# acados/acados

Measured on AMD Instinct MI355X. Metric: OCP-QP solves/sec (batch) at N=50 nx=8 nu=3, higher is better.
Workload: dtype f64; 1 GPU; random LQR OCP-QP (BASELINE configs[1]): N=50 nx=8 nu=3, u-box + x0 equality, full-space Riccati IPM, cold start, tol 1e-8, iter_max 50; batch_per_gpu=65536, global_batch=65536, parallelism=instance-sharded x1, kernel=1tpi-box<NX=8,NU=3,XBOX=0>

## Files before the change

acados_amd/csrc/gpu_batch.hip:

```cpp
#include <hip/hip_runtime.h>

#include <stdio.h>
#include <stdlib.h>
#include <string.h>

#include <algorithm>
#include <functional>
#include <string>
#include <climits>
#include <vector>

#include "acados_amd/ocp_qp_gpu_batch.h"
#include "gpu_ipm_internal.h"
#include "ipm_kernels.hpp"
#include "ipm_kernels_box.hpp"
#include "ipm_kernels_box_small.hpp"
#include "ipm_kernels_wpi.hpp"
#include "ipm_kernels_w16.hpp"
#include "ipm_kernels_w16r.hpp"
#include "ipm_kernels_w16t.hpp"
#include "ipm_kernels_wpi_mfma.hpp"
#include "res_kernels.hpp"
#include "pcond_kernels_w16.hpp"
#include "pcond_kernels_mfma.hpp"
// ... 77 lines not shown
{
    ocp_qp_gpu_batch *c = nullptr;
    int *d_list = nullptr;
    int list_cap = 0;
    int cap = 0;
};

enum BlobKind { BLOB_IN, BLOB_OUT, BLOB_VEC, BLOB_SEED, BLOB_KINDS };
struct BulkMap
{
    bool built = false;
    int len = 0, nm = 0;
    std::vector<std::string> fields;
    std::vector<int> seg_stage, seg_off, seg_len;
    std::vector<int> arr, elem;
    int *d_arr = nullptr, *d_elem = nullptr, *d_moff = nullptr, *d_mstage = nullptr, *d_mbit = nullptr;
    int *d_sgn = nullptr, *d_elem2 = nullptr;
    int *d_arr_g = nullptr, *d_elem_g = nullptr;
    gqp::GArrTable T;
};

struct HeldDynamics
{
    int tiles_invariant = 0, fact_launches = 0, rhs_launches = 0;
    hipEvent_t ev = nullptr;
    ocp_qp_gpu_batch *b = nullptr;
    bool enabled = false;
    bool polish = false;
    enum { DETECTING, AWAITING, COUNTED } state = COUNTED;
    int tiles = 0;

    void begin(ocp_qp_gpu_batch *root, hipStream_t s, bool polish_loop);
    int bits(bool affine_sweep = false) const { return !enabled ? 0 : (affine_sweep && state == DETECTING) ? 3 : 1; }
    void after_detect(hipStream_t s);
    void before_factor();
    void count();
    bool all_held() const;
    void end(hipStream_t s);
};

struct ocp_qp_gpu_batch
{
    int B = 0, Bp = 0, N = 0, device = 0;
    std::vector<int> nx, nu, nbx, nbu, nb, ng, ns, nbxe;
    std::vector<std::vector<int>> idxb, idxs_rev, idxe;
    std::vector<std::vector<int>> perm;
    bool finalized = false;
    bool use_box = false;
    int aos = 0;
    int AW = 1;
    int wpi = 0;
    bool wpi_mfma = false;
    int w16 = 0;
    size_t shmem = 0;
    size_t shmem_fwd = 0;
    size_t shmem_fact = 0;
    bool w16_soft = false;
    int w16_ng = 0;
    KernelSet wpi_ks;
    int w16_slots = 0;
    size_t w16_shmem = 0;
// ... 60 lines not shown
    int cond_N = 0;
    int cond_keep_iterate = 0;
    int force_NX = 0, force_NU = 0;
    std::vector<int> user_blocks;
    int pcond_state = 0;
    ocp_qp_gpu_batch *child = nullptr;
    const PcondSet *pc = nullptr;
    int pc_rt = 0;
    int pc_lane_expand = 0;
    const PcondzSet *pcz = nullptr;
    int pcz_mfma = 1;
    size_t pc_shmem = 0;
    std::vector<int> blk_start;
    gqp::PcondMap pmap;
    double time_xcond = 0.0;
    bool lhs_ready = false;
    SubBatch sub[SUB_ROLES];
    const KernelSet *force_ks = nullptr;
    int compact_min = 1 << 30;
    int tail_max = 12288;
    int tail_div = 4;
    int n_tail_switches = 0;
    int hold_dynamics = 1;
    HeldDynamics held;
    bool factor_stale = false;
    bool sens_open = false;
    GArr sfix = {nullptr, 0, 0};
    int *d_saved_status = nullptr;
    int ric_alg = 1;
    struct Ric1
    {
        bool saved = false;
        KernelSet own_ks;
        int w16 = 0;
        kern_redo_t w16_solve = nullptr;
        bool wpi_mfma = false;
        size_t shmem = 0, shmem_fwd = 0, shmem_fact = 0;
        std::string kname;
    } ric1;
    int n_compactions = 0;
    gqp::ResOut R = {{nullptr, 0, 0}, {nullptr, 0, 0}, {nullptr, 0, 0}, {nullptr, 0, 0}, {nullptr, 0, 0}, nullptr, 0};
    BulkMap blob[BLOB_KINDS];
    struct GradMap
    {
        bool built = false;
        int len = 0, olen = 0;
// ... 246 lines not shown
    D.t = garr<double>(b, (size_t) ((o_ct + RP)));
    D.rg = garr<double>(b, (size_t) ((N + 1) * n));
    D.rgs = garr<double>(b, (size_t) (o_s));
    D.rb = garr<double>(b, (size_t) ((N + 1) * NX));
    D.rd = garr<double>(b, (size_t) ((o_ct + RP)));
    D.rm = garr<double>(b, (size_t) ((o_ct + RP)));
    D.dux = garr<double>(b, (size_t) ((N + 2) * n));
    D.dsv = garr<double>(b, (size_t) (o_s));
    D.dpi = garr<double>(b, (size_t) ((N + 2) * NX));
    D.dlam = garr<double>(b, (size_t) ((o_ct + RP)));
    D.dt = garr<double>(b, (size_t) ((o_ct + RP)));
    D.pcorr = garr<double>(b, (size_t) ((o_ct + RP)));
    D.sD = garr<double>(b, (size_t) (o_s));
    D.sR = garr<double>(b, (size_t) (o_s));
    D.Lf = garr<double>(b, (size_t) ((N + 1) * NP));
    D.lf = garr<double>(b, (size_t) ((N + 1) * n));
    D.res = dalloc<double>(b, 4 * Bp);
    D.mu = dalloc<double>(b, Bp); D.smu = dalloc<double>(b, Bp);
    D.alpha = dalloc<double>(b, Bp); D.obj = dalloc<double>(b, Bp);
    D.apend = dalloc<double>(b, Bp);
    D.iter = dalloc<int>(b, Bp); D.status = dalloc<int>(b, Bp);
    D.n_active = dalloc<int>(b, 1);
    D.tile_inv = dalloc<int>(b, (size_t) Bp / 64);
    b->stat_inst = b->B < 64 ? b->B : 64;
    b->stat_rows = 0;
    D.stat = nullptr; D.stat_inst = 0; D.stat_rows = 0;
    D.perm = nullptr; D.n_perm = 0;

    const int grid = (b->B + 63) / 64;
    for (int k = 0; k <= N; k++)
    {
        for (int j = 0; j < n; j++)
        {
            const bool real = j < NU ? j < b->nu[k] : (j - NU) < b->nx[k];
            if (!real)
                hipLaunchKernelGGL(gqp::k_fill_strided, dim3(grid), dim3(64), 0, b->stream, D.RSQ, 1.0, b->B,
                                   k * NP + PK(j, j));
        }
        const GqpStage &S = b->st[k];
        const int nbg = S.nb + S.ng, nct = 2 * nbg + 2 * S.ns;
        uint64_t m[2] = {0, 0};
        for (int e = 0; e < nct; e++) m[e >> 6] |= (uint64_t) 1 << (e & 63);
        for (size_t e = 0; e < b->idxe[k].size(); e++)
        {
            const int sp = b->perm[k][b->idxe[k][e]];
            m[sp >> 6] &= ~((uint64_t) 1 << (sp & 63));
// ... 507 lines not shown
        std::vector<int> map, map2;
        GArr arr = {nullptr, 0, 0}, arr2 = {nullptr, 0, 0};
        const size_t flen = strlen(f);
        if (flen > 5 && !strcmp(f + flen - 5, "_mask"))
        {
            const int len = mask_bits(b, f, k, map);
            if (len < 0) { rc = -1; break; }
            if (len == 0) continue;
            if (src_len != len) { src = stage_in(b, data, (size_t) b->B * len, is_device); src_len = len; }
            int *dm = upload_map(b, map);
            hipLaunchKernelGGL(gqp::k_setmask, dim3(grid), dim3(64), 0, b->stream, src, b->B, len, dm, b->D.amask, k, b->AW);
            continue;
        }
        const int len = field_map(b, f, k, map, &arr, &map2, &arr2);
        if (len < 0)
        {
            if (stage < 0) continue;
            rc = -1;
            break;
        }
        if (len == 0) continue;
        if (src_len != len) { src = stage_in(b, data, (size_t) b->B * len, is_device); src_len = len; }
        int *dm = upload_map(b, map);
        hipLaunchKernelGGL(gqp::k_scatter, dim3(grid), dim3(64), 0, b->stream, src, b->B, len, dm, arr);
        if (arr2.p)
        {
            dm = upload_map(b, map2);
            hipLaunchKernelGGL(gqp::k_scatter, dim3(grid), dim3(64), 0, b->stream, src, b->B, len, dm, arr2);
        }
    }
    HIPCHK(hipEventRecord(e1, b->stream));
    HIPCHK(hipStreamSynchronize(b->stream));
    float ms = 0.f;
    HIPCHK(hipEventElapsedTime(&ms, e0, e1));
    b->time_pack += ms * 1e-3;
    HIPCHK(hipEventDestroy(e0)); HIPCHK(hipEventDestroy(e1));
    if (rc) fprintf(stderr, "acados_amd: ocp_qp_gpu_batch_set: unknown field %s (stage %d)\n", f, stage);
    return rc;
}
catch (const gqp_hip_failure &) { return -1; }

static void ric_switch(ocp_qp_gpu_batch *b, int v)
{
    b->ric_alg = v;
    for (SubBatch &sb : b->sub) { ocp_qp_gpu_batch_destroy(sb.c); sb.c = nullptr; }
    b->factor_stale = true;
// ... 39 lines not shown
    else if (!strcmp(f, "reg_prim")) o.reg_prim = *d;
    else if (!strcmp(f, "cond_pred_corr")) o.cond_pred_corr = *i;
    else if (!strcmp(f, "print_level")) b->print_level = *i;
    else if (!strcmp(f, "profile")) b->profile = *i;
    else if (!strcmp(f, "cond_keep_iterate")) b->cond_keep_iterate = *i;
    else if (!strcmp(f, "marker"))
    {
        typedef void (*marker_t)(int *);
        static const marker_t mk[16] = {gqp::k_marker<0>, gqp::k_marker<1>, gqp::k_marker<2>, gqp::k_marker<3>, gqp::k_marker<4>,
                                        gqp::k_marker<5>, gqp::k_marker<6>, gqp::k_marker<7>, gqp::k_marker<8>, gqp::k_marker<9>,
                                        gqp::k_marker<10>, gqp::k_marker<11>, gqp::k_marker<12>, gqp::k_marker<13>,
                                        gqp::k_marker<14>, gqp::k_marker<15>};
        HIPCHK(hipSetDevice(b->device));
        hipLaunchKernelGGL(mk[*i & 15], dim3(1), dim3(64), 0, b->stream, (int *) nullptr);
        HIPCHK(hipStreamSynchronize(b->stream));
    }
    else if (!strcmp(f, "stream_priority"))
    {
        set_stream_priority(b, *i);
    }
    else if (!strcmp(f, "compact_min")) b->compact_min = *i;
    else if (!strcmp(f, "tail_max")) b->tail_max = *i;
    else if (!strcmp(f, "hold_dynamics")) b->hold_dynamics = *i != 0;
    else if (!strcmp(f, "tail_div")) b->tail_div = *i < 1 ? 1 : *i;
    else if (!strcmp(f, "solve_max")) b->solve_max = *i;
    else if (!strcmp(f, "cond_N"))
    {
        if (*i != b->cond_N)
        {
            b->cond_N = *i;
            b->user_blocks.clear();
            b->pcond_state = 0;
            if (b->child) { ocp_qp_gpu_batch_destroy(b->child); b->child = nullptr; }
        }
    }
    else if (!strcmp(f, "cond_block_size"))
    {
        const int N2 = b->cond_N;
        if (N2 <= 0 || N2 >= b->N) { fprintf(stderr, "acados_amd: cond_block_size needs cond_N in 1..N-1 first\n"); return -1; }
        int sum = 0;
        for (int j = 0; j <= N2; j++) sum += i[j];
        bool ok = sum == b->N && i[N2] >= 0;
        for (int j = 0; j < N2; j++) ok = ok && i[j] >= 1;
        if (!ok)
        {
            fprintf(stderr, "acados_amd: partial condensing: block sizes must be >= 1 (the last one >= 0) and sum to N = %d (got %d)\n", b->N, sum);
// ... 180 lines not shown
            kp[rc] = k;
            rp[rc] = op < b->nb[k] ? b->perm[k][op] : op;
        }
        h_kp.insert(h_kp.end(), kp.begin(), kp.end());
        h_rp.insert(h_rp.end(), rp.begin(), rp.end());
        h_off[j + 1] = h_off[j] + nrow;
    }
    auto up = [&](const std::vector<int> &v) {
        int *d = dalloc<int>(b, std::max<size_t>(1, v.size()));
        if (!v.empty()) HIPCHK(hipMemcpy(d, v.data(), sizeof(int) * v.size(), hipMemcpyHostToDevice));
        return d;
    };
    int *d_start = up(b->blk_start), *d_kp = up(h_kp), *d_rp = up(h_rp), *d_off = up(h_off);
    b->pmap.gk_off = up(h_gk); b->pmap.g_rp = up(h_grp); b->pmap.g_var = up(h_gvar);
    b->pmap.slk_off = up(h_soff); b->pmap.slk_kp = up(h_skp); b->pmap.slk_sp = up(h_ssp);
    b->pmap.blk_start = d_start; b->pmap.row_kp = d_kp; b->pmap.row_rp = d_rp; b->pmap.row_off = d_off; b->pmap.N2 = N2;
    b->child = c;
    b->pcond_state = 1;
}

static void pcond_launch(ocp_qp_gpu_batch *b, bool expand)
{
    ocp_qp_gpu_batch *c = b->child;
    if (!expand && b->pcz && b->pc_rt && b->AW <= 1 && c->AW <= 1)
    {
        const dim3 grid((b->B + 3) / 4, b->pmap.N2 + 1);
        if (b->pcz_mfma)
            GQP_LAUNCH_COOP(b->pcz->cond_m, dim3((b->B + KM_PCOND_THREADS / 16 - 1) / (KM_PCOND_THREADS / 16), b->pmap.N2 + 1), dim3(KM_PCOND_THREADS), 0,
                            b->stream, b->D, c->D, b->pmap);
        else GQP_LAUNCH_COOP(b->pcz->cond, grid, dim3(64), b->pcz->shmem, b->stream, b->D, c->D, b->pmap);
        return;
    }
    if ((b->pc_rt || b->AW > 1 || c->AW > 1) && !(expand && b->pc_lane_expand && b->AW <= 1 && c->AW <= 1))
    {
        if (expand) GQP_LAUNCH_COOP(gqp::kw_pexpand, dim3(b->Bp, b->pmap.N2 + 1), dim3(64), 4 * 64 * sizeof(double), b->stream, b->D, c->D, b->pmap);
        else GQP_LAUNCH_COOP(gqp::kw_pcond, dim3(b->Bp), dim3(64), b->pc_shmem, b->stream, b->D, c->D, b->pmap);
    }
    else
    {
        const kern_pcond_t kern = expand ? b->pc->expand : b->pc->cond;
        hipLaunchKernelGGL(kern, dim3((b->B + 63) / 64), dim3(64), 0, b->stream, b->D, c->D, b->pmap);
    }
}

static int pcond_solve(ocp_qp_gpu_batch *b, int mode = 3)
{
// ... 131 lines not shown
        for (int pv = 0; pv < 64; pv++)
            if ((S.bmask >> pv) & 1)
            {
                if (!((S.emask >> pv) & 1)) { h[S.o_ct + sp] = k * 128 + sp; h[S.o_ct + nbg + sp] = k * 128 + nbg + sp; }
                sp++;
            }
        for (int g = 0; g < S.ng; g++) { h[S.o_ct + S.nb + g] = k * 128 + S.nb + g; h[S.o_ct + nbg + S.nb + g] = k * 128 + nbg + S.nb + g; }
        for (int q = 0; q < 2 * S.ns; q++) h[S.o_ct + 2 * nbg + q] = k * 128 + 2 * nbg + q;
    }
    b->d_side_map = dalloc<int>(b, h.size());
    HIPCHK(hipMemcpy(b->d_side_map, h.data(), sizeof(int) * h.size(), hipMemcpyHostToDevice));
    return b->d_side_map;
}

#ifndef GQP_HOLD_SYNC
#define GQP_HOLD_SYNC 0
#endif

void HeldDynamics::begin(ocp_qp_gpu_batch *root, hipStream_t s, bool polish_loop)
{
    b = root;
    polish = polish_loop;
    enabled = b->hold_dynamics && b->use_box && !b->wpi && !b->w16;
    state = enabled ? DETECTING : COUNTED;
    tiles = 0;
    HIPCHK(hipMemsetAsync(b->D.tile_inv, 0, sizeof(int) * (size_t) (b->Bp / 64), s));
}

void HeldDynamics::after_detect(hipStream_t s)
{
    if (state != DETECTING) return;
    HIPCHK(hipMemcpyAsync(b->h_ints, b->D.tile_inv, sizeof(int) * (size_t) (b->Bp / 64), hipMemcpyDeviceToHost, s));
    if (!ev) HIPCHK(hipEventCreate(&ev));
    HIPCHK(hipEventRecord(ev, s));
    state = AWAITING;
#if GQP_HOLD_SYNC
    HIPCHK(hipStreamSynchronize(s));
    count();
#endif
}

void HeldDynamics::before_factor()
{
    if (state != AWAITING) return;
#if defined(__HIPCC__)
    HIPCHK(hipEventSynchronize(ev));
#endif
    count();
}

void HeldDynamics::count()
{
    tiles = 0;
    for (int q = 0; q < (b->B + 63) / 64; q++) tiles += b->h_ints[q] == std::min(64, b->B - 64 * q);
    if (!polish) tiles_invariant = tiles;
    state = COUNTED;
}

bool HeldDynamics::all_held() const { return enabled && state == COUNTED && tiles == (b->B + 63) / 64; }

void HeldDynamics::end(hipStream_t s)
{
    if (b) HIPCHK(hipMemsetAsync(b->D.tile_inv, 0, sizeof(int) * (size_t) (b->Bp / 64), s));
}

static void run_ipm(ocp_qp_gpu_batch *b, ocp_qp_gpu_batch *root, Prof &prof, hipStream_t s, int it, bool polish)
{
    const IpmKernels K = pick_kernels(b);
    const bool top = b == root;
    GqpDev D = b->D;
    GqpOpts O = effective_opts(root->O, root);
    const char *eext = getenv("ACADOS_AMD_EXT_UPDATE");
    const bool ext_update = b->w16 && (eext ? atoi(eext) != 0 : (b->w16_ng > 0 || (b->B <= 16384 && b->N >= 50)));
    HeldDynamics none;
    HeldDynamics &H = top ? root->held : none;
    if (top) H.begin(root, s, polish);
    O.hold = H.bits();
    GqpOpts Oc = O;
    Oc.ext_update = ext_update ? 1 : 0;
    const int *smap = ext_update ? side_map(b) : nullptr;
    b->w16_slots = b->B;
    const char *eperm = getenv("ACADOS_AMD_W16_PERM");
    const bool use_perm = b->w16 && !(eperm && atoi(eperm) == 0);
    if (top && b->w16 && b->w16_solve && b->B <= root->solve_max && !D.perm)
    {
        prof.timed(1, s, true, [&] { launch_sweep(b, Sweep{b->w16_solve, b->w16_shmem}, s, D, O, 0); });
        root->launches++;
        root->n_single_launch++;
        HIPCHK(hipMemcpyAsync(b->h_nact, D.n_active, sizeof(int), hipMemcpyDeviceToHost, s));
        HIPCHK(hipStreamSynchronize(s));
        if (*b->h_nact <= 0)
        {
            H.end(s);
            return;
        }
    }
    for (;; it++)
    {
        H.before_factor();
        const bool all_held = H.all_held();
        const bool fact_held = all_held && K.fact_held.fn, rhs_held = all_held && K.rhs_held.fn;
        prof.timed(1, s, top, [&] { launch_sweep(b, fact_held ? K.fact_held : K.fact, s, D, O, 0); });
        if (fact_held) H.fact_launches++;
        root->launches++;
        HIPCHK(hipMemcpyAsync(b->h_nact, D.n_active, sizeof(int), hipMemcpyDeviceToHost, s));
        HIPCHK(hipStreamSynchronize(s));
        const int nact = *b->h_nact;
        if (root->print_level > 1) printf("acados_amd: ipm iter %d level size %d active %d\n", it, b->B, nact);
        if (nact <= 0 || it > O.iter_max) break;
        if (use_perm && nact >= 1 && 6 * nact <= 5 * b->w16_slots)
        {
            if (!b->d_perm) { b->d_perm = dalloc<int>(b, b->Bp); b->d_perm_cnt = dalloc<int>(b, 1); }
            HIPCHK(hipMemsetAsync(b->d_perm_cnt, 0, sizeof(int), s));
            hipLaunchKernelGGL(gqp::k_active_perm, dim3((b->B + 255) / 256), dim3(256), 0, s, D, b->d_perm, b->d_perm_cnt);
            D.perm = b->d_perm;
            D.n_perm = nact;
            b->w16_slots = nact;
        }
        if (!b->wpi && root->tail_max > 0 && nact <= root->tail_max && (long) root->tail_div * nact <= b->B)
        {
            ocp_qp_gpu_batch *tail = compact_into(b, root, s, SUB_TAIL);
            root->n_tail_switches++;
            run_ipm(tail, root, prof, s, it);
            launch_whole(tail, pick_kernels(tail).final_, s, tail->D);
            root->launches++;
            compact_back(b, s, SUB_TAIL, it);
            break;
        }
        if (b->B >= root->compact_min && 2 * nact <= b->B)
        {
            ocp_qp_gpu_batch *level = compact_into(b, root, s, SUB_COMPACT);
            root->n_compactions++;
            run_ipm(level, root, prof, s, it);
            compact_back(b, s, SUB_COMPACT, it);
            break;
        }
        GqpOpts Oa = O;
        Oa.hold = H.bits(true);
        prof.timed(2, s, top, [&] { launch_sweep(b, K.faff, s, D, Oa, 0); });
        H.after_detect(s);
        const Sweep &k_rhs = rhs_held ? K.rhs_held : K.rhs;
        prof.timed(3, s, top, [&] { launch_sweep(b, k_rhs, s, D, O, 0); });
        prof.timed(4, s, top, [&] { launch_sweep(b, K.fcorr, s, D, Oc, 0); });
        root->launches += 3;
        if (O.cond_pred_corr)
        {
            launch_sweep(b, k_rhs, s, D, O, 1);
            launch_sweep(b, K.fcorr, s, D, Oc, 1);
            root->launches += 2;
        }
        if (rhs_held) H.rhs_launches += O.cond_pred_corr ? 2 : 1;
        if (ext_update)
        {
            const int blocks = D.ux.aos ? b->B : (b->B + GQP_UPD_THREADS - 1) / GQP_UPD_THREADS;
            hipLaunchKernelGGL(gqp::k_step_update, dim3(blocks), dim3(GQP_UPD_THREADS), 0, s, D, O, smap, b->nct_tot, b->ns2_tot);
            root->launches++;
        }
    }
    b->w16_slots = b->B;
    H.end(s);
}

static void polish_pass(ocp_qp_gpu_batch *b, Prof &prof, hipStream_t s)
// ... 104 lines not shown
    return c;
}

static void sub_batch_opts(const ocp_qp_gpu_batch *from, ocp_qp_gpu_batch *c, SubRole role)
{
    c->O = from->O;
    c->tol_comp_soft_scale = from->tol_comp_soft_scale;
    if (role != SUB_RIC0) return;
    c->polish = from->polish; c->polish_ratio = from->polish_ratio; c->polish_min = from->polish_min;
    c->print_level = from->print_level; c->profile = from->profile; c->compact_min = from->compact_min; c->solve_max = from->solve_max;
    c->t0_min = from->t0_min; c->lam0_min = from->lam0_min;
}

static void sub_copy(ocp_qp_gpu_batch *b, const SubBatch &sb, const std::vector<GqpArrMember> &arrays, int cnt, int dir, hipStream_t s)
{
    for (GqpArrMember m : arrays) copy_level(b->D.*m, sb.c->D.*m, sb.d_list, cnt, dir, s);
}

static void sub_batch_load(ocp_qp_gpu_batch *b, const SubBatch &sb, int cnt, hipStream_t s)
{
    ocp_qp_gpu_batch *c = sb.c;
    c->B = cnt;
    c->D.B = cnt;
    sub_copy(b, sb, g_state_arrays, cnt, 0, s);
    copy_level(b->D.amask, c->D.amask, sb.d_list, cnt, 0, s);
    hipLaunchKernelGGL(gqp::k_compact_scalars, dim3((cnt + 63) / 64), dim3(64), 0, s, b->D, c->D, sb.d_list, cnt, 0);
    HIPCHK(hipStreamSynchronize(s));
}

static void sub_batch_store(ocp_qp_gpu_batch *b, const SubBatch &sb, int cnt, SubStore what, hipStream_t s)
{
    sub_copy(b, sb, what == SUB_RESULT ? g_result_arrays : what == SUB_DIRECTION ? g_direction_arrays : g_factor_arrays, cnt, 1, s);
    if (what == SUB_RESULT)
        hipLaunchKernelGGL(gqp::k_compact_scalars, dim3((cnt + 63) / 64), dim3(64), 0, s, b->D, sb.c->D, sb.d_list, cnt, 1);
}

static ocp_qp_gpu_batch *compact_into(ocp_qp_gpu_batch *b, ocp_qp_gpu_batch *root, hipStream_t s, SubRole role)
{
    const bool tail = role == SUB_TAIL;
    SubBatch &sb = b->sub[role];
    int *st = b->h_ints, *list = b->h_ints + b->Bp;
    HIPCHK(hipMemcpy(st, b->D.status, sizeof(int) * b->B, hipMemcpyDeviceToHost));
    int cnt = 0;
    for (int i = 0; i < b->B; i++) if (st[i] == GQP_RUNNING) list[cnt++] = i;
    sub_list_reserve(b, sb, std::max(cnt, (b->Bp + 1) / 2));
    if (sb.c && cnt > (tail ? sb.cap : sb.c->Bp))
// ... 153 lines not shown
int ocp_qp_gpu_batch_solve(ocp_qp_gpu_batch *b)
try
{
    HIPCHK(hipSetDevice(b->device));
    finalize_structure(b);
    if (b->full_dense) return dense_solve(b);
    if (b->cond_N > 0 && b->cond_N < b->N)
    {
        if (b->pcond_state == 0) pcond_setup(b);
        if (b->pcond_state == 1) return pcond_solve(b, b->lhs_ready ? 2 : 3);
    }
    if (b->ric_alg == 0 && !b->wpi) return ric0_solve(b);
    b->time_xcond = 0.0;
    ensure_stat(b);
    const KernelSet *ks = b->ks;
    GqpDev D = b->D;
    GqpOpts O = effective_opts(b->O, b);
    const dim3 grid((b->B + 63) / 64), block(64);
    hipStream_t s = b->stream;
    b->launches = 0;
    b->n_compactions = 0;
    b->n_tail_switches = 0;
    b->n_single_launch = 0;
    b->held.tiles_invariant = b->held.rhs_launches = b->held.fact_launches = 0;
    b->prof_cls.clear();
    Prof prof;
    prof.root = b;

    HIPCHK(hipEventRecord(b->ev0, s));
    *b->h_nact = b->B;
    HIPCHK(hipMemcpyAsync(D.n_active, b->h_nact, sizeof(int), hipMemcpyHostToDevice, s));
    if (D.stat) HIPCHK(hipMemsetAsync(D.stat, 0, sizeof(double) * (size_t) b->stat_rows * GQP_STAT_COLS * b->stat_inst, s));
    if (O.warm_start < 2)
    {
        prof.timed(0, s, true, [&] { launch_whole(b, ks->init, s, D, O); });
        b->launches++;
    }
    else
    {
        const double clip = O.warm_start == 2 ? 0.1 : 0.0;
        hipLaunchKernelGGL(gqp::k_hot_start, grid, block, 0, s, D, std::max(clip, b->t0_min), std::max(clip, b->lam0_min));
        b->launches++;
    }
    HIPCHK(hipMemsetAsync(D.apend, 0, sizeof(double) * (size_t) b->Bp, s));
    run_ipm(b, b, prof, s, 0);
    b->n_polished = b->n_polish_reverted = 0;
    if (b->polish) polish_pass(b, prof, s);
// ... 314 lines not shown
    std::vector<double> h((size_t) b->stat_rows * GQP_STAT_COLS * b->stat_inst);
    HIPCHK(hipMemcpy(h.data(), b->D.stat, sizeof(double) * h.size(), hipMemcpyDeviceToHost));
    for (int r = 0; r < rows; r++)
        for (int c = 0; c < GQP_STAT_COLS; c++)
            stat[r * GQP_STAT_COLS + c] = h[((size_t) r * GQP_STAT_COLS + c) * b->stat_inst + inst];
    return rows;
}
catch (const gqp_hip_failure &) { return -1; }

double ocp_qp_gpu_batch_get_scalar(ocp_qp_gpu_batch *b, const char *f)
try
{
    if (!strcmp(f, "time_tot")) return b->time_tot;
    if (!strcmp(f, "time_pack")) { double t = b->time_pack; b->time_pack = 0.0; return t; }
    if (!strcmp(f, "iter_max_batch")) return (double) b->last_iters;
    if (!strcmp(f, "launches")) return (double) b->launches;
    if (!strcmp(f, "time_xcond")) return b->time_xcond;
    if (!strcmp(f, "compactions")) return (double) b->n_compactions;
    if (!strcmp(f, "w16_tiles")) return (double) b->w16_tiles;
    if (!strcmp(f, "tail_switches")) return (double) b->n_tail_switches;
    if (!strcmp(f, "tiles_invariant")) return (double) b->held.tiles_invariant;
    if (!strcmp(f, "rhs_held_launches")) return (double) b->held.rhs_launches;
    if (!strcmp(f, "fact_held_launches")) return (double) b->held.fact_launches;
    if (!strcmp(f, "single_launch_solves")) return (double) b->n_single_launch;
    if (!strcmp(f, "cond_N_active")) return b->pcond_state == 1 ? (double) b->child->N : (double) b->N;
    if (!strcmp(f, "tol_comp_soft_scale")) return b->tol_comp_soft_scale;
    if (!strcmp(f, "polish")) return b->polish;
    if (!strcmp(f, "full_dense")) return b->full_dense;
    if (!strcmp(f, "dense_columns")) return b->kd.nv;
    if (!strcmp(f, "dense_workspace_bytes")) return (double) b->kd.W * 8.0 * b->kd_slice;
    if (!strcmp(f, "polished")) return b->child && b->pcond_state == 1 && b->cond_N > 0 && b->cond_N < b->N ? b->child->n_polished : b->n_polished;
    if (!strcmp(f, "polish_reverted")) return b->child && b->pcond_state == 1 && b->cond_N > 0 && b->cond_N < b->N ? b->child->n_polish_reverted : b->n_polish_reverted;
    if (!strcmp(f, "tol_comp_effective")) { finalize_structure(b); return effective_opts(b->O, b).tol_comp; }
    if (!strcmp(f, "pcond_kernel")) return b->pcond_state != 1 ? -1.0 : (b->pcz && b->pc_rt && b->AW <= 1 && b->child->AW <= 1) ? (b->pcz_mfma ? 3.0 : 2.0) : b->pc_rt ? 0.0 : 1.0;
    if (!strcmp(f, "pexpand_kernel")) return b->pcond_state != 1 ? -1.0 : (!b->pc_rt || b->pc_lane_expand) ? 1.0 : 0.0;
    {
        const char *cls[6] = {"init", "back_fact", "fwd_aff", "back_rhs", "fwd_corr", "finalize"};
        for (int q = 0; q < 6; q++)
        {
            char nm[64];
            snprintf(nm, sizeof(nm), "prof_ms_%s", cls[q]);
            if (!strcmp(f, nm)) return b->prof_ms[q];
            snprintf(nm, sizeof(nm), "prof_cnt_%s", cls[q]);
            if (!strcmp(f, nm)) return (double) b->prof_cnt[q];
        }
        if (!strcmp(f, "prof_reset"))
// ... 110 lines not shown
try
{
    const int bad = ocp_qp_gpu_batch_solve(b);
    b->lhs_ready = false;
    return bad;
}
catch (const gqp_hip_failure &) { return -1; }


static const char *const k_bulk_in_fields[] = {"A", "B", "b", "Q", "S", "R", "q", "r", "lbu", "ubu", "lbx", "ubx", "lg", "ug",
                                               "C", "D", "Zl", "Zu", "zl", "zu", "lls", "lus", "lbu_mask", "ubu_mask",
                                               "lbx_mask", "ubx_mask", "lg_mask", "ug_mask", "lls_mask", "lus_mask"};
static const char *const k_bulk_out_fields[] = {"u", "x", "sl", "su", "pi", "lam", "t"};
static const char *const k_bulk_vec_fields[] = {"b", "q", "r", "lbu", "ubu", "lbx", "ubx", "lg", "ug", "zl", "zu", "lls", "lus", "lbu_mask", "ubu_mask",
                                                "lbx_mask", "ubx_mask", "lg_mask", "ug_mask", "lls_mask", "lus_mask"};
static const char *const k_seed_fields[] = {"r", "q", "zl", "zu", "b", "lbu", "lbx", "lg", "ubu", "ubx", "ug", "lls", "lus"};

struct BlobDesc
{
    const char *const *fields;
    int nf;
    const char *prefix;
    bool masks, read_map;
};
#define GQP_BLOB(fields, prefix, masks, read_map) {fields, (int) (sizeof(fields) / sizeof(fields[0])), prefix, masks, read_map}
static const BlobDesc k_blobs[BLOB_KINDS] = {
     GQP_BLOB(k_bulk_in_fields, "", true, true),
     GQP_BLOB(k_bulk_out_fields, "", false, false),
     GQP_BLOB(k_bulk_vec_fields, "", true, false),
     GQP_BLOB(k_seed_fields, "seed_", false, false),
};

static BlobKind blob_kind(int v, bool has_out = true)
{
    if (v == 2) return BLOB_VEC;
    return v && has_out ? BLOB_OUT : BLOB_IN;
}

struct BlobField
{
    const char *f;
    int k, len;
    bool is_mask;
    std::vector<int> map, map2;
    GArr arr = {nullptr, 0, 0}, arr2 = {nullptr, 0, 0};
};

static void blob_open_segment(BulkMap &M, const std::string &name, int k, int len)
{
    M.fields.push_back(name); M.seg_stage.push_back(k); M.seg_off.push_back((int) M.arr.size()); M.seg_len.push_back(len);
}

static void blob_fields(ocp_qp_gpu_batch *b, const BlobDesc &K, const std::function<void(const BlobField &)> &visit)
// ... 127 lines not shown

static void bulk_gather_launch(ocp_qp_gpu_batch *b, double *dst, int len, const int *d_arr, const int *d_elem, const gqp::GArrTable &T)
{
    if (b->aos && !getenv("ACADOS_AMD_SCATTER_PLAIN"))
        hipLaunchKernelGGL(gqp::k_bulk_gather_aos, dim3((len + 255) / 256, b->B), dim3(256), 0, b->stream, dst, b->B, len, d_arr, d_elem, T);
    else if (!getenv("ACADOS_AMD_SCATTER_PLAIN"))
        GQP_LAUNCH_COOP(gqp::k_bulk_gather_tile, dim3((b->B + 63) / 64, (len + 63) / 64), dim3(64), 0, b->stream, dst, b->B, len, d_arr, d_elem, T);
    else
        hipLaunchKernelGGL(gqp::k_bulk_gather, dim3((b->B + 63) / 64, (len + 255) / 256), dim3(64), 0, b->stream, dst, b->B, len, d_arr, d_elem, T);
}

static void bulk_scatter_launch(ocp_qp_gpu_batch *b, const double *src, int len, BulkMap &M)
{
    if (b->aos && !getenv("ACADOS_AMD_SCATTER_PLAIN"))
        hipLaunchKernelGGL(gqp::k_bulk_scatter_aos, dim3((len + 255) / 256, b->B), dim3(256), 0, b->stream, src, b->B, len, M.d_arr, M.d_elem, M.T);
    else if (!getenv("ACADOS_AMD_SCATTER_PLAIN"))
        GQP_LAUNCH_COOP(gqp::k_bulk_scatter_tile, dim3((b->B + 63) / 64, (len + 63) / 64), dim3(64), 0, b->stream, src, b->B, len, M.d_arr, M.d_elem, M.T);
    else
        hipLaunchKernelGGL(gqp::k_bulk_scatter, dim3((b->B + 63) / 64, (len + 255) / 256), dim3(64), 0, b->stream, src, b->B, len, M.d_arr, M.d_elem, M.T);
}

static void blob_scatter(ocp_qp_gpu_batch *b, BulkMap &M, const double *src)
{
    bulk_scatter_launch(b, src, M.len, M);
    if (M.nm)
        hipLaunchKernelGGL(gqp::k_bulk_masks, dim3((b->B + 63) / 64, (b->N + 1 + GQP_MASK_SPC - 1) / GQP_MASK_SPC), dim3(64), 0, b->stream, src, b->B, M.len, M.d_moff,
                           M.d_mstage, M.d_mbit, M.nm, b->D.amask, b->AW, GQP_MASK_SPC);
}

static void blob_set(ocp_qp_gpu_batch *b, BlobKind kind, const double *blob, int is_device)
{
    BulkMap &M = blob_map(b, kind);
    pack_timed(b, [&] { blob_scatter(b, M, stage_in(b, blob, (size_t) b->B * M.len, is_device)); });
}

int ocp_qp_gpu_batch_set_bulk(ocp_qp_gpu_batch *b, const double *blob, int is_device)
try
{
    blob_set(b, BLOB_IN, blob, is_device);
    return 0;
}
catch (const gqp_hip_failure &) { return -1; }

int ocp_qp_gpu_batch_set_bulk_vec(ocp_qp_gpu_batch *b, const double *blob, int is_device)
try
{
// ... 619 lines not shown
```

acados_amd/csrc/ipm_kernels_box.hpp:

```cpp
#ifndef IPM_KERNELS_BOX_HPP_
#define IPM_KERNELS_BOX_HPP_

#include "ipm_kernels.hpp"

namespace gqp
{

__device__ static inline double frcp(double x)
{
#if defined(__HIP_DEVICE_COMPILE__)
    double r = __builtin_amdgcn_rcp(x);
    double e = __builtin_fma(-x, r, 1.0);
    r = __builtin_fma(r, e, r);
    e = __builtin_fma(-x, r, 1.0);
    return __builtin_fma(r, e, r);
#else
    return 1.0 / x;
#endif
}

__device__ static inline double frsqrt(double x)
{
#if defined(__HIP_DEVICE_COMPILE__)
    double y = __builtin_amdgcn_rsq(x);
// ... 515 lines not shown
    const int i = blockIdx.x * blockDim.x + threadIdx.x;
    const bool run = i < D.B && D.status[i] == GQP_RUNNING;
    if (!GQP_WAVE_ANY(run)) return;

    constexpr int NBL = GQP_KH_BROWS_LDS < NU ? GQP_KH_BROWS_LDS : NU;
    static_assert((NX + NBL) * NX * 64 * 8 <= 40 * 1024, "4 single-wave blocks per CU must fit");
    __shared__ double Al[(NX + NBL) * NX * 64];
#define GQP_KH_LDS(r) ((r) < NBL || (r) >= NU)
#define GQP_KH_SLOT(r) ((r) < NBL ? (r) : (r) >= NU ? NBL + (r) - NU : 0)
#define GQP_KH_REG(r) ((r) >= NBL && (r) < NU ? (r) - NBL : 0)
    const int lane_w = threadIdx.x;
    int lane_r = threadIdx.x;
    GQP_OPAQUE(lane_r);
    double Bt[(NU - NBL > 0 ? NU - NBL : 1) * NX];
    UNROLL for (int e = 0; e < (NU - NBL) * NX; e++) Bt[e] = 0.0;
    TileTab tiles;
#define GQP_KH_PUT(name) tiles.template put<KH_##name>(tile_ptr(D.name));
    GQP_KH_ARRAYS(GQP_KH_PUT)
#undef GQP_KH_PUT
    tiles.template put<KH_COUNT>((double *) D.n_active);
    tiles.template put<KH_COUNT + 1>((double *) D.status);
    tiles.template put<KH_COUNT + 2>(D.stat);
    tiles.template put<KH_COUNT + 3>((double *) (((uint64_t) (unsigned int) D.stat_rows << 32) | (unsigned int) D.stat_inst));
#define KACC(name, e0) acc_tile(tiles.get(KH_##name + zs), (size_t) (e0), i)
    double Lx[NPX], lx[NX];
    UNROLL for (int e = 0; e < NPX; e++) Lx[e] = 0.0;
    UNROLL for (int c = 0; c < NX; c++) lx[c] = 0.0;
    double nrm_g = 0.0, nrm_b = 0.0, nrm_d = 0.0, nrm_m = 0.0, musum = 0.0, obj = 0.0;
    int nact = 0;
    double xn[NX], pin[NX];
    UNROLL for (int c = 0; c < NX; c++) { xn[c] = 0.0; pin[c] = 0.0; }
#if GQP_KB_FOLD
    const double apd = run ? D.apend[i] : 0.0;
    const bool pend = apd != 0.0;
#endif

    for (int k = D.N; k >= 0; k--)
    {
        const StageU S = stage_u(D.st, k);
        const uint64_t imask = S.bmask & ~S.emask;
        const uint64_t am = GAT(D.amask, k);
        const int nbg = S.nb;
        int ord = 0;
        int zs = 0;
        GQP_OPAQUE_S(zs);

// ... 106 lines not shown
        UNROLL for (int q = 0; q < NX; q++)
        {
            double w[n];
            UNROLL for (int r = 0; r < n; r++)
            {
                if (GQP_KH_LDS(r) && GQP_KH_SLOT(r) % GQP_KH_LROWS == 0 && r >= GQP_KH_LAHEAD) GQP_AFTER(lr, w[r - GQP_KH_LAHEAD]);
                double a = 0.0;
                UNROLL for (int p = q; p < NX; p++)
                    a += (GQP_KH_LDS(r) ? Al[(GQP_KH_SLOT(r) * NX + p) * 64 + lr] : Bt[GQP_KH_REG(r) * NX + p]) * Lx[PK(p, q)];
                w[r] = a;
            }
            UNROLL for (int r = 0; r < n; r++)
            {
                mm[r] += w[r] * w0[q];
                UNROLL for (int c = 0; c < r; c++) M[PK(r, c)] += w[r] * w[c];
                double wd = w[r];
                if (r >= NU + 2) GQP_OPAQUE_D(wd);
                M[PK(r, r)] += w[r] * wd;
            }
        }
        UNROLL for (int r = 0; r < n; r++) mm[r] = mm[r] + (r < NB ? gadd[r < NB ? r : 0] : 0.0);

        UNROLL for (int r = 0; r < n; r++) hv[r] = 0.0;
        const Acc aRSQ = KACC(RSQ, k * NP);
        double H[GQP_HROW_CHUNK * n];
        UNROLL for (int r = 0; r < n; r++)
        {
            if (r % GQP_HROW_CHUNK == 0)
            {
                GQP_AFTER(ord, M[r > 0 ? PK(r - 1, r - 1) : NP - 1]);
                UNROLL for (int r2 = r; r2 < n && r2 < r + GQP_HROW_CHUNK; r2++)
                    UNROLL for (int c = 0; c <= r2; c++) H[(r2 % GQP_HROW_CHUNK) * n + c] = aRSQ.ldjo(0, PK(r2, c), ord);
            }
            double *const h = H + (r % GQP_HROW_CHUNK) * n;
            UNROLL for (int c = 0; c < r; c++)
            {
                hv[r] += h[c] * v[c];
                hv[c] += h[c] * v[r];
            }
            hv[r] += h[r] * v[r];
            h[r] += O.reg_prim + (r < NB ? gam[r < NB ? r : 0] : 0.0);
            UNROLL for (int c = 0; c <= r; c++) M[PK(r, c)] = h[c] + M[PK(r, c)];
        }
        UNROLL for (int r = 0; r < n; r++)
        {
            obj += (0.5 * hv[r] + g[r]) * v[r];
            gt[r] += hv[r] + g[r];
// ... 79 lines not shown
    }
    int status = GQP_RUNNING;
    const bool bad = nrm_g != nrm_g || nrm_b != nrm_b || nrm_d != nrm_d || nrm_m != nrm_m || mu != mu;
    if (bad) status = 1;
    else if (nrm_g <= O.tol_stat && nrm_b <= O.tol_eq && nrm_d <= O.tol_ineq && nrm_m <= O.tol_comp) status = 0;
    else if (it >= O.iter_max) status = 2;
    else if (dabs(D.alpha[i]) <= O.alpha_min) status = 3;
    if (status != GQP_RUNNING)
    {
        status_p[i] = status;
        atomicSub(n_active_p, 1);
    }
}
#undef KACC
#undef GQP_KH_LDS
#undef GQP_KH_SLOT
#undef GQP_KH_REG

template <int NX, int NU>
constexpr auto kh_factor_for() -> void (*)(GqpDev, GqpOpts, int)
{
    if constexpr (kb_hold<NX, NU, false>() && NX == 8 && NU == 3) return kh_factor<NX, NU>;
    else return nullptr;
}


template <int NX, int NU, bool XBOX>
__global__ void __launch_bounds__(64) kb_backrhs(GqpDev D, GqpOpts O, int redo)
{
    constexpr int n = NX + NU, NP = n * (n + 1) / 2, NPX = NX * (NX + 1) / 2, NB = XBOX ? n : NU;
    const int i = blockIdx.x * blockDim.x + threadIdx.x;
    if (i >= D.B) return;
    const bool run = D.status[i] == GQP_RUNNING;
    if (redo ? !(run && D.alpha[i] < 0.0) : !GQP_WAVE_ANY(run)) return;
    const double smu = D.smu[i];
    const double pscale = redo ? 0.0 : 1.0;

    double Lx[NPX], lx[NX];
    UNROLL for (int e = 0; e < NPX; e++) Lx[e] = 0.0;
    UNROLL for (int c = 0; c < NX; c++) lx[c] = 0.0;

    for (int k = D.N; k >= 0; k--)
    {
        const StageU S = stage_u(D.st, k);
        const uint64_t imask = S.bmask & ~S.emask;
        const uint64_t am = GAT(D.amask, k);
// ... 466 lines not shown
```

profiles/summarize.py:

```python
#!/usr/bin/env python3
import sqlite3
import sys


def kernel_src_hash():
    import glob, hashlib, os
    root = os.path.join(os.path.dirname(os.path.dirname(os.path.abspath(__file__))), "acados_amd", "csrc")
    h = hashlib.sha256()
    for f in sorted(glob.glob(os.path.join(root, "*.hpp")) + glob.glob(os.path.join(root, "*.hip")) + glob.glob(os.path.join(root, "*.h")) + glob.glob(os.path.join(root, "*.cpp"))):
        h.update(os.path.basename(f).encode())
        h.update(open(f, "rb").read())
    return h.hexdigest()[:16]


def kernel(db):
    cur = sqlite3.connect(db).cursor()
    print(f"{'kernel':80s} {'calls':>6s} {'total_us':>12s} {'avg_us':>10s} {'pct':>6s}")
    for name, calls, tot, avg, pct in cur.execute("select name,total_calls,total_duration,average,percentage from top_kernels"):
        print(f"{name[:80]:80s} {calls:6d} {tot:12.1f} {avg:10.1f} {pct:6.2f}")
    print("\nper-dispatch durations of the IPM kernels (us), in launch order, first 60:")
    rows = cur.execute("select name,duration,vgpr_count,accum_vgpr_count,sgpr_count,scratch_size from kernels "
                       "where name like '%gqp::k_backward%' or name like '%gqp::k_forward%' or name like '%gqp::kb_%' or name like '%gqp::kh_%' "
                       "or name like '%gqp::kw_%' or name like '%gqp::kx_%' or name like '%gqp::ky_%' or name like '%gqp::kz_%' order by start limit 60").fetchall()
    for name, dur, v, a, s, sc in rows:
        short = name.split("gqp::")[1].split("(")[0]
        print(f"  {short:40s} {dur / 1e3:10.1f}  vgpr {v} agpr {a} sgpr {s} scratch {sc}")


def timeline(db, which=-1):
    cur = sqlite3.connect(db).cursor()
    rows = cur.execute("select name,start,end from kernels order by start").fetchall()
    marks = [i for i, r in enumerate(rows) if "_init<" in r[0] or "k_init" in r[0]]
    if len(marks) < 2:
        print("fewer than two solves in the trace"); return
    which = int(which)
    lo, hi = (marks[which - 1], marks[which]) if which < 0 else (marks[which], marks[which + 1])
    while lo > 0 and rows[lo - 1][1] > rows[lo][1] - 3e6 and "finalize" not in rows[lo - 1][0] and "pexpand" not in rows[lo - 1][0]:
        lo -= 1
    t0, prev_end, busy = rows[lo][1], rows[lo][1], 0.0
    print(f"{'offset_us':>10s} {'dur_us':>9s} {'gap_us':>8s}  kernel")
    for name, st, en in rows[lo:hi]:
        short = name.split("gqp::")[1].split("(")[0] if "gqp::" in name else name[:40]
        print(f"{(st - t0) / 1e3:10.1f} {(en - st) / 1e3:9.1f} {(st - prev_end) / 1e3:8.1f}  {short}")
        busy += (en - st) / 1e3
        prev_end = max(prev_end, en)
# ... 130 lines not shown
```

Measured before the change: 1.505 million OCP-QP solves/s.

## Reuse stage-invariant Hessian and cache dynamics-invariance detection across solves

Adds a per-tile detector that checks whether the cost Hessian RSQ is bitwise identical across all stages. When it is, the held factorization kernel reads one stage's RSQ for every stage, cutting global memory traffic. The dynamics-invariance detection result is kept with a data-version counter, so repeated solves on unchanged data skip the detecting sweep and its host round-trip. In exchange there is version bookkeeping on every data write, an extra detector kernel with a host sync whenever the Hessian data changes, and a risk of stale verdicts if some write path does not bump the version.

New measurement: 1.621 million OCP-QP solves/s, median of 6. 1.08x the previous value.

```diff
diff --git a/acados_amd/csrc/gpu_batch.hip b/acados_amd/csrc/gpu_batch.hip
--- a/acados_amd/csrc/gpu_batch.hip
+++ b/acados_amd/csrc/gpu_batch.hip
@@ -123,8 +123,17 @@
 
 struct HeldDynamics
 {
-    int tiles_invariant = 0, fact_launches = 0, rhs_launches = 0;
+    int tiles_invariant = 0, fact_launches = 0, rhs_launches = 0, hess_launches = 0, hess_detects = 0, detects = 0;
     hipEvent_t ev = nullptr;
+    unsigned ver_dyn = 1, ver_hess = 1;
+    unsigned kept_at = 0;
+    int kept_tiles = 0;
+    int *d_kept = nullptr;
+    unsigned hess_at = 0;
+    bool hess_inv = false;
+    int *d_hess_cnt = nullptr;
+    unsigned pending_ver = 0;
+    bool complete = false;
     ocp_qp_gpu_batch *b = nullptr;
     bool enabled = false;
     bool polish = false;
@@ -133,11 +142,14 @@
 
     void begin(ocp_qp_gpu_batch *root, hipStream_t s, bool polish_loop);
     int bits(bool affine_sweep = false) const { return !enabled ? 0 : (affine_sweep && state == DETECTING) ? 3 : 1; }
-    void after_detect(hipStream_t s);
-    void before_factor();
+    void after_detect(hipStream_t s, bool all_running);
+    void before_factor(bool fact_entry);
+    void stream_drained();
     void count();
     bool all_held() const;
+    bool hessian_verdict(hipStream_t s);
     void end(hipStream_t s);
+    void data_written(bool dyn, bool hess) { if (dyn) ver_dyn++; if (hess) ver_hess++; if (!ver_dyn) ver_dyn = 1; if (!ver_hess) ver_hess = 1; }
 };
 
 struct ocp_qp_gpu_batch
@@ -244,6 +256,7 @@
     int tail_div = 4;
     int n_tail_switches = 0;
     int hold_dynamics = 1;
+    int hold_hessian = 1;
     HeldDynamics held;
     bool factor_stale = false;
     bool sens_open = false;
@@ -536,6 +549,8 @@
     D.iter = dalloc<int>(b, Bp); D.status = dalloc<int>(b, Bp);
     D.n_active = dalloc<int>(b, 1);
     D.tile_inv = dalloc<int>(b, (size_t) Bp / 64);
+    b->held.d_kept = dalloc<int>(b, (size_t) Bp / 64);
+    b->held.d_hess_cnt = dalloc<int>(b, (size_t) Bp / 64);
     b->stat_inst = b->B < 64 ? b->B : 64;
     b->stat_rows = 0;
     D.stat = nullptr; D.stat_inst = 0; D.stat_rows = 0;
@@ -1089,6 +1104,7 @@
         if (len == 0) continue;
         if (src_len != len) { src = stage_in(b, data, (size_t) b->B * len, is_device); src_len = len; }
         int *dm = upload_map(b, map);
+        b->held.data_written(arr.p == b->D.BAt.p, arr.p == b->D.RSQ.p);
         hipLaunchKernelGGL(gqp::k_scatter, dim3(grid), dim3(64), 0, b->stream, src, b->B, len, dm, arr);
         if (arr2.p)
         {
@@ -1174,6 +1190,7 @@
     else if (!strcmp(f, "compact_min")) b->compact_min = *i;
     else if (!strcmp(f, "tail_max")) b->tail_max = *i;
     else if (!strcmp(f, "hold_dynamics")) b->hold_dynamics = *i != 0;
+    else if (!strcmp(f, "hold_hessian")) b->hold_hessian = *i != 0;
     else if (!strcmp(f, "tail_div")) b->tail_div = *i < 1 ? 1 : *i;
     else if (!strcmp(f, "solve_max")) b->solve_max = *i;
     else if (!strcmp(f, "cond_N"))
@@ -1400,6 +1417,7 @@
 static void pcond_launch(ocp_qp_gpu_batch *b, bool expand)
 {
     ocp_qp_gpu_batch *c = b->child;
+    if (!expand) c->held.data_written(true, true);
     if (!expand && b->pcz && b->pc_rt && b->AW <= 1 && c->AW <= 1)
     {
         const dim3 grid((b->B + 3) / 4, b->pmap.N2 + 1);
@@ -1577,15 +1595,31 @@
     b = root;
     polish = polish_loop;
     enabled = b->hold_dynamics && b->use_box && !b->wpi && !b->w16;
+    pending_ver = 0;
+    const size_t bytes = sizeof(int) * (size_t) (b->Bp / 64);
+    if (enabled && !polish && kept_at == ver_dyn)
+    {
+        state = COUNTED;
+        tiles = tiles_invariant = kept_tiles;
+        HIPCHK(hipMemcpyAsync(b->D.tile_inv, d_kept, bytes, hipMemcpyDeviceToDevice, s));
+        return;
+    }
     state = enabled ? DETECTING : COUNTED;
     tiles = 0;
-    HIPCHK(hipMemsetAsync(b->D.tile_inv, 0, sizeof(int) * (size_t) (b->Bp / 64), s));
-}
-
-void HeldDynamics::after_detect(hipStream_t s)
+    HIPCHK(hipMemsetAsync(b->D.tile_inv, 0, bytes, s));
+}
+
+void HeldDynamics::after_detect(hipStream_t s, bool all_running)
 {
     if (state != DETECTING) return;
     HIPCHK(hipMemcpyAsync(b->h_ints, b->D.tile_inv, sizeof(int) * (size_t) (b->Bp / 64), hipMemcpyDeviceToHost, s));
+    if (!polish)
+    {
+        HIPCHK(hipMemcpyAsync(d_kept, b->D.tile_inv, sizeof(int) * (size_t) (b->Bp / 64), hipMemcpyDeviceToDevice, s));
+        pending_ver = ver_dyn;
+        complete = all_running;
+        detects++;
+    }
     if (!ev) HIPCHK(hipEventCreate(&ev));
     HIPCHK(hipEventRecord(ev, s));
     state = AWAITING;
@@ -1595,9 +1629,10 @@
 #endif
 }
 
-void HeldDynamics::before_factor()
+void HeldDynamics::before_factor(bool fact_entry)
 {
     if (state != AWAITING) return;
+    if (!fact_entry) return;
 #if defined(__HIPCC__)
     HIPCHK(hipEventSynchronize(ev));
 #endif
@@ -1610,9 +1645,37 @@
     for (int q = 0; q < (b->B + 63) / 64; q++) tiles += b->h_ints[q] == std::min(64, b->B - 64 * q);
     if (!polish) tiles_invariant = tiles;
     state = COUNTED;
+    if (pending_ver && (complete || tiles == (b->B + 63) / 64))
+    {
+        kept_at = pending_ver;
+        kept_tiles = tiles;
+    }
+    pending_ver = 0;
+}
+
+void HeldDynamics::stream_drained()
+{
+    if (state == AWAITING) count();
 }
 
 bool HeldDynamics::all_held() const { return enabled && state == COUNTED && tiles == (b->B + 63) / 64; }
+
+bool HeldDynamics::hessian_verdict(hipStream_t s)
+{
+    if (hess_at == ver_hess) return hess_inv;
+    const int nt = (b->B + 63) / 64;
+    int *h = b->h_ints;
+    HIPCHK(hipMemsetAsync(d_hess_cnt, 0, sizeof(int) * (size_t) (b->Bp / 64), s));
+    hipLaunchKernelGGL(gqp::k_hess_invariant, dim3(nt), dim3(64), 0, s, b->D, d_hess_cnt);
+    HIPCHK(hipMemcpyAsync(h, d_hess_cnt, sizeof(int) * (size_t) nt, hipMemcpyDeviceToHost, s));
+    HIPCHK(hipStreamSynchronize(s));
+    int full = 0;
+    for (int q = 0; q < nt; q++) full += h[q] == std::min(64, b->B - 64 * q);
+    hess_inv = full == nt;
+    hess_at = ver_hess;
+    hess_detects++;
+    return hess_inv;
+}
 
 void HeldDynamics::end(hipStream_t s)
 {
@@ -1652,14 +1715,19 @@
     }
     for (;; it++)
     {
-        H.before_factor();
+        H.before_factor(K.fact_held.fn != nullptr);
         const bool all_held = H.all_held();
         const bool fact_held = all_held && K.fact_held.fn, rhs_held = all_held && K.rhs_held.fn;
-        prof.timed(1, s, top, [&] { launch_sweep(b, fact_held ? K.fact_held : K.fact, s, D, O, 0); });
+        const bool hess_held = fact_held && root->hold_hessian && H.hessian_verdict(s);
+        GqpOpts Of = O;
+        if (hess_held) Of.hold |= 4;
+        prof.timed(1, s, top, [&] { launch_sweep(b, fact_held ? K.fact_held : K.fact, s, D, Of, 0); });
         if (fact_held) H.fact_launches++;
+        if (hess_held) H.hess_launches++;
         root->launches++;
         HIPCHK(hipMemcpyAsync(b->h_nact, D.n_active, sizeof(int), hipMemcpyDeviceToHost, s));
         HIPCHK(hipStreamSynchronize(s));
+        H.stream_drained();
         const int nact = *b->h_nact;
         if (root->print_level > 1) printf("acados_amd: ipm iter %d level size %d active %d\n", it, b->B, nact);
         if (nact <= 0 || it > O.iter_max) break;
@@ -1693,7 +1761,7 @@
         GqpOpts Oa = O;
         Oa.hold = H.bits(true);
         prof.timed(2, s, top, [&] { launch_sweep(b, K.faff, s, D, Oa, 0); });
-        H.after_detect(s);
+        H.after_detect(s, nact == b->B);
         const Sweep &k_rhs = rhs_held ? K.rhs_held : K.rhs;
         prof.timed(3, s, top, [&] { launch_sweep(b, k_rhs, s, D, O, 0); });
         prof.timed(4, s, top, [&] { launch_sweep(b, K.fcorr, s, D, Oc, 0); });
@@ -1844,6 +1912,7 @@
     ocp_qp_gpu_batch *c = sb.c;
     c->B = cnt;
     c->D.B = cnt;
+    c->held.data_written(true, true);
     sub_copy(b, sb, g_state_arrays, cnt, 0, s);
     copy_level(b->D.amask, c->D.amask, sb.d_list, cnt, 0, s);
     hipLaunchKernelGGL(gqp::k_compact_scalars, dim3((cnt + 63) / 64), dim3(64), 0, s, b->D, c->D, sb.d_list, cnt, 0);
@@ -2043,7 +2112,7 @@
     b->n_compactions = 0;
     b->n_tail_switches = 0;
     b->n_single_launch = 0;
-    b->held.tiles_invariant = b->held.rhs_launches = b->held.fact_launches = 0;
+    b->held.tiles_invariant = b->held.rhs_launches = b->held.fact_launches = b->held.hess_launches = b->held.hess_detects = b->held.detects = 0;
     b->prof_cls.clear();
     Prof prof;
     prof.root = b;
@@ -2404,6 +2473,9 @@
     if (!strcmp(f, "tiles_invariant")) return (double) b->held.tiles_invariant;
     if (!strcmp(f, "rhs_held_launches")) return (double) b->held.rhs_launches;
     if (!strcmp(f, "fact_held_launches")) return (double) b->held.fact_launches;
+    if (!strcmp(f, "hess_held_launches")) return (double) b->held.hess_launches;
+    if (!strcmp(f, "hess_detector_runs")) return (double) b->held.hess_detects;
+    if (!strcmp(f, "detecting_sweeps")) return (double) b->held.detects;
     if (!strcmp(f, "single_launch_solves")) return (double) b->n_single_launch;
     if (!strcmp(f, "cond_N_active")) return b->pcond_state == 1 ? (double) b->child->N : (double) b->N;
     if (!strcmp(f, "tol_comp_soft_scale")) return b->tol_comp_soft_scale;
@@ -2560,13 +2632,14 @@
     int nf;
     const char *prefix;
     bool masks, read_map;
+    bool matrices;
 };
-#define GQP_BLOB(fields, prefix, masks, read_map) {fields, (int) (sizeof(fields) / sizeof(fields[0])), prefix, masks, read_map}
+#define GQP_BLOB(fields, prefix, masks, read_map, matrices) {fields, (int) (sizeof(fields) / sizeof(fields[0])), prefix, masks, read_map, matrices}
 static const BlobDesc k_blobs[BLOB_KINDS] = {
-     GQP_BLOB(k_bulk_in_fields, "", true, true),
-     GQP_BLOB(k_bulk_out_fields, "", false, false),
-     GQP_BLOB(k_bulk_vec_fields, "", true, false),
-     GQP_BLOB(k_seed_fields, "seed_", false, false),
+     GQP_BLOB(k_bulk_in_fields, "", true, true, true),
+     GQP_BLOB(k_bulk_out_fields, "", false, false, false),
+     GQP_BLOB(k_bulk_vec_fields, "", true, false, false),
+     GQP_BLOB(k_seed_fields, "seed_", false, false, false),
 };
 
 static BlobKind blob_kind(int v, bool has_out = true)
@@ -2740,6 +2813,8 @@
 
 static void blob_scatter(ocp_qp_gpu_batch *b, BulkMap &M, const double *src)
 {
+    const bool matrices = k_blobs[&M - b->blob].matrices;
+    b->held.data_written(matrices, matrices);
     bulk_scatter_launch(b, src, M.len, M);
     if (M.nm)
         hipLaunchKernelGGL(gqp::k_bulk_masks, dim3((b->B + 63) / 64, (b->N + 1 + GQP_MASK_SPC - 1) / GQP_MASK_SPC), dim3(64), 0, b->stream, src, b->B, M.len, M.d_moff,
diff --git a/acados_amd/csrc/ipm_kernels_box.hpp b/acados_amd/csrc/ipm_kernels_box.hpp
--- a/acados_amd/csrc/ipm_kernels_box.hpp
+++ b/acados_amd/csrc/ipm_kernels_box.hpp
@@ -561,6 +561,7 @@
     tiles.template put<KH_COUNT + 1>((double *) D.status);
     tiles.template put<KH_COUNT + 2>(D.stat);
     tiles.template put<KH_COUNT + 3>((double *) (((uint64_t) (unsigned int) D.stat_rows << 32) | (unsigned int) D.stat_inst));
+    tiles.template put<KH_COUNT + 4>((double *) (uint64_t) (unsigned int) ((O.hold & 4) ? D.N - 1 : -1));
 #define KACC(name, e0) acc_tile(tiles.get(KH_##name + zs), (size_t) (e0), i)
     double Lx[NPX], lx[NX];
     UNROLL for (int e = 0; e < NPX; e++) Lx[e] = 0.0;
@@ -713,7 +714,9 @@
         UNROLL for (int r = 0; r < n; r++) mm[r] = mm[r] + (r < NB ? gadd[r < NB ? r : 0] : 0.0);
 
         UNROLL for (int r = 0; r < n; r++) hv[r] = 0.0;
-        const Acc aRSQ = KACC(RSQ, k * NP);
+        const int hess_at = (int) (unsigned int) (uint64_t) tiles.get(KH_COUNT + 4);
+        const int kh = (hess_at >= 0 && k < D.N) ? hess_at : k;
+        const Acc aRSQ = KACC(RSQ, kh * NP);
         double H[GQP_HROW_CHUNK * n];
         UNROLL for (int r = 0; r < n; r++)
         {
@@ -839,6 +842,25 @@
 {
     if constexpr (kb_hold<NX, NU, false>() && NX == 8 && NU == 3) return kh_factor<NX, NU>;
     else return nullptr;
+}
+
+static __global__ void __launch_bounds__(64) k_hess_invariant(GqpDev D, int *cnt)
+{
+    const int i = blockIdx.x * blockDim.x + threadIdx.x;
+    if (i >= D.B) return;
+    const int n = D.NX + D.NU, NP = n * (n + 1) / 2;
+    uint64_t differs = 0;
+    for (int e = 0; e < NP; e++)
+    {
+        const uint64_t first = dbits(GAT(D.RSQ, e));
+        for (int k = 1; k < D.N; k++) differs |= first ^ dbits(GAT(D.RSQ, k * NP + e));
+    }
+#if defined(__HIP_DEVICE_COMPILE__)
+    const int same = popc64(__builtin_amdgcn_ballot_w64(differs == 0));
+    if (threadIdx.x == 0) cnt[blockIdx.x] = same;
+#else
+    if (differs == 0) cnt[blockIdx.x] += 1;
+#endif
 }
 
 
diff --git a/profiles/summarize.py b/profiles/summarize.py
--- a/profiles/summarize.py
+++ b/profiles/summarize.py
@@ -20,7 +20,7 @@
         print(f"{name[:80]:80s} {calls:6d} {tot:12.1f} {avg:10.1f} {pct:6.2f}")
     print("\nper-dispatch durations of the IPM kernels (us), in launch order, first 60:")
     rows = cur.execute("select name,duration,vgpr_count,accum_vgpr_count,sgpr_count,scratch_size from kernels "
-                       "where name like '%gqp::k_backward%' or name like '%gqp::k_forward%' or name like '%gqp::kb_%' or name like '%gqp::kh_%' "
+                       "where name like '%gqp::k_backward%' or name like '%gqp::k_forward%' or name like '%gqp::kb_%' or name like '%gqp::kh_%' or name like '%gqp::k_hess_%' "
                        "or name like '%gqp::kw_%' or name like '%gqp::kx_%' or name like '%gqp::ky_%' or name like '%gqp::kz_%' order by start limit 60").fetchall()
     for name, dur, v, a, s, sc in rows:
         short = name.split("gqp::")[1].split("(")[0]
```
